# biirving/meant

Hardware: AMD Instinct MI355X
Metric: samples/sec fwd+bwd, MEANT lag=12 d=768 (higher is better)
Workload: dtype bf16; 1 GPU; full MEANT (tweet+image) fwd+CE+bwd, lag=12, d=768, 12 heads, seq=512, 224x224 p=16, E=1, vocab 64001 (BASELINE.json configs[2]/[3]); batch_per_gpu=128, global_batch=128, parallelism=dp1, micro_batches=1, train_mode_dropout=True, activation_checkpointing=False, norm_linear_fold=False, grad_allreduce=False

## Files before the change

meant_amd/csrc/qkv_fwd_by_id.hip:

```cpp
#pragma clang fp contract(off)
#include "common.h"
#include "internal.h"

#define FBYID_REQ(c, ...) MEANT_REQUIRE(c, MEANT_ERR_ARG, __VA_ARGS__)

namespace {

#include "seg_sum.h"
constexpr int PANEL = 256;

__global__ __launch_bounds__(256) void qkv_gather_kernel(const float* __restrict__ P, const int64_t* __restrict__ sorted_ids,
                                                          const int64_t* __restrict__ order, const uint8_t* __restrict__ live,
                                                          const float* __restrict__ qa, const float* __restrict__ qb,
                                                          const float* __restrict__ ka, const float* __restrict__ kb, bf16* __restrict__ qkv,
                                                          int64_t n, int N3, int D, int Dh, int R, int S, int64_t V, int cb_chunks) {
  const int lane = threadIdx.x & 63, wave = threadIdx.x >> 6;
  const int64_t s = (int64_t)blockIdx.x * 4 + wave;
  const int64_t j0 = s * SEG;
  if (j0 >= n) return;
  const int64_t j1 = j0 + SEG < n ? j0 + SEG : n;
  const int c0 = blockIdx.y * cb_chunks;
  const int left = (N3 >> 3) - c0;
  const int nch = left < cb_chunks ? left : cb_chunks;
  const bool has = lane < nch;
  const int col = (c0 + (has ? lane : 0)) * 8;
  const int sec = col / D;
  const int c = (col - sec * D) % Dh;
  const bool rot_on = qa != nullptr && sec < 2 && c < R;
  const bool kv = sec >= 1;
  const float* const tabA = (sec == 1 ? ka : qa) + (rot_on ? c : 0);
  const float* const tabB = (sec == 1 ? kb : qb) + (rot_on ? c : 0);
  long long cur = -1;
  Vec8<float> row{};

  for (int64_t jb = j0; jb < j1; jb += 64) {
    const int64_t jl = jb + lane < j1 ? jb + lane : j1 - 1;
    const long long id64 = sorted_ids[jl], ord64 = order[jl];
    const int my_id = id64 >= 0 && id64 < V ? (int)id64 : -1;
    const int my_ord = ord64 >= 0 && ord64 < n ? (int)ord64 : -1;
    const int cnt = (int)(j1 - jb < 64 ? j1 - jb : 64);
    for (int t0 = 0; t0 < cnt; t0 += 4) {
      Vec8<float> r4[4], A4[4], B4[4];
      int ord4[4];
      bool st4[4];
#pragma unroll
      for (int u = 0; u < 4; ++u) {
        const int t = t0 + u < cnt ? t0 + u : cnt - 1;
        const int id = __builtin_amdgcn_readlane(my_id, t);
        const int ord = __builtin_amdgcn_readlane(my_ord, t);
        if (id != cur) {
          cur = id;
          if (id >= 0) row = load8<float>(P + (int64_t)id * N3 + col);
        }
        r4[u] = row;
        ord4[u] = ord;
        const bool tok = t0 + u < cnt && id >= 0 && ord >= 0;
        const bool kv_ok = !live || (tok && live[ord / PANEL] != 0);
        st4[u] = tok && has && (!kv || kv_ok);
        A4[u] = Vec8<float>{};
        B4[u] = Vec8<float>{};
        if (st4[u] && rot_on) {
          const int o = (ord % S) * R;
          A4[u] = load8<float>(tabA + o);
          B4[u] = load8<float>(tabB + o);
        }
      }
#pragma unroll
      for (int u = 0; u < 4; ++u) {
        if (!st4[u]) continue;
        float v[8];
#pragma unroll
        for (int e = 0; e < 8; ++e) v[e] = r4[u].get(e);
        if (rot_on) rot_apply8(v, A4[u].lo, A4[u].hi, B4[u].lo, B4[u].hi);
        Vec8<bf16> o;
#pragma unroll
        for (int e = 0; e < 8; ++e) o.set(e, v[e]);
        store8s<bf16>(qkv + (int64_t)ord4[u] * N3 + col, o);
      }
    }
  }
}

struct FwdByIdWs { size_t ntab, rinv, p, live, total; };
FwdByIdWs fwd_byid_layout(int64_t n, int64_t d, int64_t N3, int64_t V) {
  FwdByIdWs w;
  const int64_t Vp = vpad_rows(V);
  size_t off = 0;
  const auto take = [&off](size_t bytes) { const size_t o = off; off += align256(bytes); return o; };
  w.ntab = take((size_t)Vp * d * sizeof(bf16));
  w.rinv = take((size_t)V * sizeof(float));
  w.p = take((size_t)Vp * N3 * sizeof(float));
  w.live = take((size_t)ceil_div(n, PANEL));
  w.total = off;
  return w;
}

bool fwd_byid_shape_ok(int64_t n, int64_t d, int64_t N3, int64_t V) {
  return n > 0 && d > 0 && N3 > 0 && V > 0 && n < (1ll << 31) && V < (1ll << 31) && d % 8 == 0 && N3 % 24 == 0 && N3 < (1ll << 22) && d < (1ll << 22);
}

GemmBf16Args shape_args(int64_t M, int64_t N, int64_t K) { return gemm_bf16_nt_args(nullptr, K, nullptr, nullptr, N, M, N, K); }

}

extern "C" size_t meant_qkv_embed_fwd_by_id_ws(int64_t n, int64_t d, int64_t N3, int64_t V) {
  return fwd_byid_shape_ok(n, d, N3, V) ? fwd_byid_layout(n, d, N3, V).total : 0;
}

extern "C" int meant_qkv_embed_fwd_by_id_ok(int64_t n, int64_t d, int64_t N3, int64_t V) {
  if (!fwd_byid_shape_ok(n, d, N3, V) || N3 % 3 != 0 || (N3 / 3) % 256 != 0 || n % 256 != 0) return 0;
  if (meant_num_cus() <= 0) return 0;
  const int64_t Vp = vpad_rows(V);
  return gemm_bf16_nt_streams(shape_args(n, N3, d)) && gemm_bf16_nt_streams(shape_args(Vp, N3, d)) ? 1 : 0;
}

extern "C" int meant_qkv_embed_fwd_by_id(const void* table_bf16, const float* gain, float eps, const void* w_bf16, const float* bias,
                                         const int64_t* sorted_ids, const int64_t* order, const void* kv_lists, const float* qa,
                                         const float* qb, const float* ka, const float* kb, void* qkv, int64_t n, int64_t S, int64_t d,
                                         int H, int Dh, int R, int64_t V, void* workspace, size_t workspace_bytes, void* stream) {
  FBYID_REQ(table_bf16 && gain && w_bf16 && sorted_ids && order && qkv && workspace && H > 0 && Dh > 0 && S > 0, "qkv_embed_fwd_by_id: bad argument");
  const int64_t D = (int64_t)H * Dh, N3 = 3 * D;
  MEANT_REQUIRE(fwd_byid_shape_ok(n, d, N3, V) && n % S == 0 && S < (1ll << 22) && Dh % 8 == 0, MEANT_ERR_UNSUPPORTED,
                "qkv_embed_fwd_by_id: n=%lld S=%lld d=%lld H=%d Dh=%d V=%lld: n, V < 2^31, n %% S == 0, d %% 8 == 0, Dh %% 8 == 0", (long long)n,
                (long long)S, (long long)d, H, Dh, (long long)V);
  const bool rot = qa != nullptr;
  FBYID_REQ(!rot || (qb && ka && kb && R > 0 && R % 8 == 0 && R <= Dh), "qkv_embed_fwd_by_id: bad rotary tables (rot_dim %% 8 == 0)");
  MEANT_REQUIRE(meant_qkv_embed_fwd_by_id_ok(n, d, N3, V), MEANT_ERR_UNSUPPORTED,
                "qkv_embed_fwd_by_id: the streaming NT kernel must take both the [n, H Dh] and the [V, 3 H Dh] product (n=%lld d=%lld N3=%lld V=%lld)",
                (long long)n, (long long)d, (long long)N3, (long long)V);
  const FwdByIdWs w = fwd_byid_layout(n, d, N3, V);
  MEANT_REQUIRE(workspace_bytes >= w.total, MEANT_ERR_WORKSPACE, "qkv_embed_fwd_by_id: workspace of %zu bytes needed, %zu given", w.total,
                workspace_bytes);
  FBYID_REQ(meant_aligned16(workspace) && meant_aligned16(table_bf16) && meant_aligned16(w_bf16) && meant_aligned16(qkv) &&
                (!rot || (meant_aligned16(qa) && meant_aligned16(qb) && meant_aligned16(ka) && meant_aligned16(kb))),
            "qkv_embed_fwd_by_id: 16-byte alignment");
  const bool listed = kv_lists != nullptr;
  FBYID_REQ(!listed || S % PANEL == 0, "qkv_embed_fwd_by_id: key-padding lists need S %% 256 == 0");
  hipStream_t st = (hipStream_t)stream;
  char* base = (char*)workspace;
  bf16* ntab = (bf16*)(base + w.ntab);
  float *rinv = (float*)(base + w.rinv), *P = (float*)(base + w.p);
  uint8_t* live = listed ? (uint8_t*)(base + w.live) : nullptr;
  const int64_t Vp = vpad_rows(V), nst = ceil_div(n, SEG), nblk = n / 64, npan = n / PANEL;

  const int64_t V4 = V & ~(int64_t)3;
  int rc = meant_rmsnorm_fwd(table_bf16, gain, ntab, rinv, V4, d, eps, 0.f, 0, MEANT_BF16, stream);
  if (!rc && V4 < V)
    rc = meant_rmsnorm_fwd((const bf16*)table_bf16 + (V - 4) * d, gain, ntab + (V - 4) * d, rinv + (V - 4), 4, d, eps, 0.f, 0, MEANT_BF16, stream);
  if (rc) return rc;
  hipError_t e = hipSuccess;
  if (Vp > V) e = hipMemsetAsync(ntab + V * d, 0, (size_t)(Vp - V) * d * sizeof(bf16), st);
  if (e == hipSuccess && listed) e = hipMemsetAsync(live, 0, (size_t)npan, st);
  MEANT_REQUIRE(e == hipSuccess, MEANT_ERR_LAUNCH, "qkv_embed_fwd_by_id: clearing the workspace failed: %s", hipGetErrorString(e));
  GemmBf16Args a{};
  a.A = ntab; a.lda = d; a.B = (const bf16*)w_bf16; a.ldb = d; a.C = (bf16*)P; a.ldc = N3;
  a.M = Vp; a.N = N3; a.K = d; a.bias = bias; a.epilogue = GEMM_EPI_F32_OUT;
  rc = gemm_bf16_nt_launch(a, st);
  if (rc) return rc;
  const int* const lists = (const int*)kv_lists;
  if (listed) rc = live_flags_launch(lists + MEANT_KV_LIST_HDR + nblk, lists + 1, live, npan, st);
  if (rc) return rc;
  const SegColBlocks cb = seg_col_blocks(N3, 1);
  hipLaunchKernelGGL(qkv_gather_kernel, dim3((unsigned)ceil_div(nst, 4), (unsigned)cb.ncb), dim3(256), 0, st, (const float*)P, sorted_ids, order,
                     (const uint8_t*)live, qa, qb, ka, kb, (bf16*)qkv, n, (int)N3, (int)D, Dh, rot ? R : 0, (int)S, V, cb.cb_chunks);
  MEANT_LAUNCH_CHECK("qkv_embed_fwd_by_id: gather");
  meant_route_hit(ROUTE_QKV_FWD_BY_ID);
  if (listed) return zero_panels_launch((bf16*)qkv + D, N3, 2 * D, lists + MEANT_KV_LIST_HDR + nblk + npan, lists + 2, npan, st);
  return MEANT_OK;
}
```

meant_amd/csrc/seg_sum.h:

```cpp
#pragma once

constexpr int SEG = 256;
constexpr int SEG_SHORT = 16;

struct SegAddRow {
  float* dtable; int64_t id_lo, id_hi;
  __device__ __forceinline__ bool owns(int64_t id) const { return id >= id_lo && id < id_hi; }
  __device__ __forceinline__ void put(int64_t id, int64_t ld, int64_t col, f32x4 a) const {
    f32x4* dst = reinterpret_cast<f32x4*>(dtable + id * ld + col);
    *dst = *dst + a;
  }
};
struct SegStoreHiLo {
  bf16* hi; bf16* lo;
  __device__ __forceinline__ bool owns(int64_t) const { return true; }
  __device__ __forceinline__ void put(int64_t id, int64_t ld, int64_t col, f32x4 a) const {
    bf16x4 h, l;
#pragma unroll
    for (int e = 0; e < 4; ++e) {
      h[e] = (bf16)a[e];
      l[e] = (bf16)(a[e] - (float)h[e]);
    }
    *reinterpret_cast<bf16x4*>(hi + id * ld + col) = h;
    *reinterpret_cast<bf16x4*>(lo + id * ld + col) = l;
  }
};

struct SegAllRows {
  __device__ __forceinline__ bool live(int64_t) const { return true; }
  __device__ __forceinline__ bool reads(int, bool) const { return true; }
};
template <class Store>
struct SegSlotSink {
  Store st; float* part; int64_t ld;
  __device__ __forceinline__ bool owns(int64_t id) const { return st.owns(id); }
  __device__ __forceinline__ void inside(int64_t id, int64_t col, f32x4 lo, f32x4 hi) const {
    st.put(id, ld, col, lo);
    st.put(id, ld, col + 4, hi);
  }
  __device__ __forceinline__ void cross(int64_t, int slot, int64_t col, f32x4 lo, f32x4 hi) const {
    store8<float>(part + slot * ld + col, Vec8<float>{lo, hi});
  }
};

struct SegCols { int64_t col[2]; bool has[2]; };
__device__ __forceinline__ SegCols seg_cols(int64_t width, int cb_chunks) {
  const int lane = threadIdx.x & 63;
  const int c0 = blockIdx.y * cb_chunks;
  const int left = (int)(width >> 3) - c0;
  const int nch = left < cb_chunks ? left : cb_chunks;
  return {{(int64_t)(c0 + lane) * 8, (int64_t)(c0 + lane + 64) * 8}, {lane < nch, lane + 64 < nch}};
}

template <bool COLSUM, typename T, class Rows, class Sink>
__device__ __forceinline__ void seg_walk(const T* __restrict__ src, int64_t ld, const int64_t* __restrict__ sorted_ids,
                                         const int64_t* __restrict__ order, int64_t n, int64_t V, int64_t j0, int64_t j1, const SegCols& c,
                                         const Rows& rows, const Sink& sink, float* __restrict__ csum) {
  const int lane = threadIdx.x & 63;
  float acc[2][8], cs[2][8];
#pragma unroll
  for (int e = 0; e < 8; ++e) acc[0][e] = acc[1][e] = cs[0][e] = cs[1][e] = 0.f;
  int64_t cur = sorted_ids[j0];
  bool open_left = j0 > 0 && sorted_ids[j0 - 1] == cur;

  auto flush = [&](int64_t id, int slot) {
    if (id < 0 || id >= V || !sink.owns(id)) return;
#pragma unroll
    for (int k = 0; k < 2; ++k) {
      if (!c.has[k]) continue;
      const f32x4 lo = {acc[k][0], acc[k][1], acc[k][2], acc[k][3]}, hi = {acc[k][4], acc[k][5], acc[k][6], acc[k][7]};
      if (slot < 0) sink.inside(id, c.col[k], lo, hi);
      else sink.cross(id, slot, c.col[k], lo, hi);
    }
  };

  for (int64_t jb = j0; jb < j1; jb += 64) {
    const int64_t jl = jb + lane < j1 ? jb + lane : j1 - 1;
    const long long my_id = sorted_ids[jl], my_ord = order[jl];
    const int cnt = (int)(j1 - jb < 64 ? j1 - jb : 64);
    for (int t0 = 0; t0 < cnt; t0 += 4) {
      Vec8<T> r[4][2];
      long long ids4[4];
#pragma unroll
      for (int u = 0; u < 4; ++u) {
        const int t = t0 + u < cnt ? t0 + u : cnt - 1;
        ids4[u] = __shfl(my_id, t, 64);
        const long long ord = __shfl(my_ord, t, 64);
        const bool row_ok = ord >= 0 && ord < n;
        const bool live = row_ok && rows.live(ord);
        const T* row = src + (row_ok ? ord : 0) * ld;
#pragma unroll
        for (int k = 0; k < 2; ++k) {
          r[u][k] = Vec8<T>{};
          if (c.has[k] && row_ok && rows.reads(k, live)) r[u][k] = load8s<T>(row + c.col[k]);
        }
      }
#pragma unroll
      for (int u = 0; u < 4; ++u) {
        if (t0 + u >= cnt) break;
        const int64_t id = ids4[u];
        if (id != cur) {
          flush(cur, open_left ? 0 : -1);
#pragma unroll
          for (int e = 0; e < 8; ++e) acc[0][e] = acc[1][e] = 0.f;
          cur = id;
          open_left = false;
        }
#pragma unroll
        for (int e = 0; e < 8; ++e) {
#pragma unroll
          for (int k = 0; k < 2; ++k) {
            const float a = r[u][k].get(e);
            acc[k][e] += a;
            if constexpr (COLSUM) cs[k][e] += a;
          }
        }
      }
    }
  }
  const bool open_right = j1 < n && sorted_ids[j1] == cur;
  flush(cur, open_left ? 0 : (open_right ? 1 : -1));
  if constexpr (COLSUM) {
#pragma unroll
    for (int k = 0; k < 2; ++k)
      if (c.has[k])
        store8<float>(csum + c.col[k], Vec8<float>{{cs[k][0], cs[k][1], cs[k][2], cs[k][3]}, {cs[k][4], cs[k][5], cs[k][6], cs[k][7]}});
  }
}

template <class Store>
__global__ __launch_bounds__(256) void seg_cross_kernel(const int64_t* __restrict__ sorted_ids, const float* __restrict__ part,
                                                         int* __restrict__ longk, Store st, int64_t n, int64_t d, int64_t V) {
  const int lane = threadIdx.x & 63, wave = threadIdx.x >> 6;
  const int64_t s = (int64_t)blockIdx.x * 4 + wave, j0 = s * SEG, j1 = j0 + SEG;
  if (j1 >= n) return;
  const int64_t id = sorted_ids[j1 - 1];
  const bool owner = sorted_ids[j1] == id && !(j0 > 0 && sorted_ids[j0 - 1] == id)
                     && id >= 0 && id < V && st.owns(id);
  int64_t K = 0;
  if (owner) {
    const int64_t nst = (n + SEG - 1) / SEG;
    int64_t follow = 0;
    for (int64_t t0 = s + 1;; t0 += 64) {
      const int64_t t = t0 + lane;
      const int k = __popcll(__ballot(t < nst && sorted_ids[t * SEG] == id));
      follow += k;
      if (k < 64) break;
    }
    K = follow + 1;
  }
  if (blockIdx.y == 0 && lane == 0) longk[s] = K > SEG_SHORT ? (int)K : 0;
  if (K == 0 || K > SEG_SHORT) return;
  const int64_t col = (int64_t)blockIdx.y * 256 + lane * 4;
  if (col >= d) return;
  f32x4 acc = *reinterpret_cast<const f32x4*>(part + (s * 2 + 1) * d + col);
  for (int64_t k = 1; k < K; ++k) acc += *reinterpret_cast<const f32x4*>(part + (s + k) * 2 * d + col);
  st.put(id, d, col, acc);
}

template <class Store>
__global__ __launch_bounds__(256) void seg_long_kernel(const int64_t* __restrict__ sorted_ids, const float* __restrict__ part,
                                                        const int* __restrict__ longk, Store st, int64_t d) {
  __shared__ f32x4 red[16][16];
  const int tid = threadIdx.x;
  const int64_t s = blockIdx.x;
  const int64_t K = longk[s];
  if (K == 0) return;
  const int64_t id = sorted_ids[s * SEG + SEG - 1];
  const int p = tid >> 4;
  const int64_t col = (int64_t)blockIdx.y * 64 + (tid & 15) * 4;
  const bool active = col < d;
  const int64_t piece = (K + 15) / 16, k0 = p * piece, k1 = k0 + piece < K ? k0 + piece : K;
  f32x4 acc = {0.f, 0.f, 0.f, 0.f};
  if (active) {
#pragma unroll 4
    for (int64_t k = k0; k < k1; ++k) {
      const float* row = k == 0 ? part + (s * 2 + 1) * d : part + (s + k) * 2 * d;
      acc += *reinterpret_cast<const f32x4*>(row + col);
    }
  }
  red[p][tid & 15] = acc;
  __syncthreads();
#pragma unroll
  for (int h = 8; h > 0; h >>= 1) {
    if (p < h) red[p][tid & 15] += red[p + h][tid & 15];
    __syncthreads();
  }
  if (p == 0 && active) st.put(id, d, col, red[0][tid & 15]);
}

struct SegColBlocks { int ncb, cb_chunks; };
inline SegColBlocks seg_col_blocks(int64_t width, int per_lane) {
  const int64_t chunks = width >> 3, ncb = ceil_div(chunks, 64 * per_lane);
  return {(int)ncb, (int)ceil_div(chunks, ncb)};
}

template <class Store>
void seg_cross_launch(const Store& store, const int64_t* sorted_ids, const float* part, int* longk, int64_t n, int64_t d, int64_t V,
                      hipStream_t st) {
  const int64_t nst = ceil_div(n, SEG);
  if (nst <= 1) return;
  hipLaunchKernelGGL(seg_cross_kernel<Store>, dim3((unsigned)ceil_div(nst - 1, 4), (unsigned)ceil_div(d, 256)), dim3(256), 0, st, sorted_ids,
                     part, longk, store, n, d, V);
  hipLaunchKernelGGL(seg_long_kernel<Store>, dim3((unsigned)(nst - 1), (unsigned)ceil_div(d, 64)), dim3(256), 0, st, sorted_ids, part,
                     (const int*)longk, store, d);
}
```

Baseline: 3812 samples/s.

## Software-pipeline gather and segment-sum walks with double-buffered loads

Restructures the QKV gather kernel and the shared seg_walk helper into a software pipeline. The next group of row loads, and the index block after that, are requested before the current group is stored or accumulated, with liveness flags precomputed per lane. The gather gains a specialised no-rotary path with unconditional row loads, uses segment indices made wave-uniform, and rounds column blocks to multiples of 8. The intent is to hide global-load latency in these memory-bound gather and reduce passes, at the cost of more registers and branchless dummy loads.

```diff
diff --git a/meant_amd/csrc/qkv_fwd_by_id.hip b/meant_amd/csrc/qkv_fwd_by_id.hip
--- a/meant_amd/csrc/qkv_fwd_by_id.hip
+++ b/meant_amd/csrc/qkv_fwd_by_id.hip
@@ -8,6 +8,101 @@
 
 #include "seg_sum.h"
 constexpr int PANEL = 256;
+
+constexpr int GATHER_G = 2;
+struct GatherBlock { int id, ord, off, kv_ok; };
+template <bool ROT>
+struct GatherSet;
+template <>
+struct GatherSet<true> { Vec8<float> r[GATHER_G], A[GATHER_G], B[GATHER_G]; int ord[GATHER_G]; bool st[GATHER_G]; };
+template <>
+struct GatherSet<false> { Vec8<float> r[GATHER_G]; int ord[GATHER_G]; bool st[GATHER_G]; };
+inline SegColBlocks gather_col_blocks(int64_t width) {
+  const SegColBlocks cb = seg_col_blocks(width, 1);
+  const int cut = (cb.cb_chunks + 7) & ~7;
+  return {(int)ceil_div(width >> 3, cut), cut};
+}
+
+template <bool ROT>
+__device__ __forceinline__ void gather_walk(const float* __restrict__ P, const int64_t* __restrict__ sorted_ids, const int64_t* __restrict__ order,
+                                            const uint8_t* __restrict__ live, const float* __restrict__ tabA, const float* __restrict__ tabB,
+                                            bf16* __restrict__ qkv, int64_t n, int N3, int R, int S, int64_t V, int64_t j0, int64_t j1, int col,
+                                            bool has, bool kv, bool rot_on) {
+  const int lane = threadIdx.x & 63;
+  int cur = -1;
+  Vec8<float> row{};
+
+  auto entries = [&](int64_t jb) {
+    const int64_t jl = jb + lane < j1 ? jb + lane : j1 - 1;
+    const long long id64 = sorted_ids[jl], ord64 = order[jl];
+    GatherBlock b;
+    b.id = id64 >= 0 && id64 < V ? (int)id64 : -1;
+    b.ord = ord64 >= 0 && ord64 < n ? (int)ord64 : -1;
+    b.off = b.ord >= 0 ? (b.ord % S) * R : 0;
+    b.kv_ok = 1;
+    return b;
+  };
+  auto flags = [&](const GatherBlock& b) { return !live || (b.ord >= 0 && live[b.ord / PANEL] != 0) ? 1 : 0; };
+  auto request = [&](const GatherBlock& b, int t0, int cnt, GatherSet<ROT>& g) {
+#pragma unroll
+    for (int u = 0; u < GATHER_G; ++u) {
+      const int t = t0 + u < cnt ? t0 + u : (cnt ? cnt - 1 : 0);
+      const int id = __builtin_amdgcn_readlane(b.id, t);
+      const int ord = __builtin_amdgcn_readlane(b.ord, t);
+      g.ord[u] = ord;
+      g.st[u] = t0 + u < cnt && id >= 0 && ord >= 0 && has && (!kv || __builtin_amdgcn_readlane(b.kv_ok, t) != 0);
+      if constexpr (ROT) {
+        if (id != cur) {
+          cur = id;
+          if (id >= 0) row = load8<float>(P + (int64_t)id * N3 + col);
+        }
+        g.r[u] = row;
+        const int o = __builtin_amdgcn_readlane(b.off, t);
+        g.A[u] = load8<float>(tabA + o);
+        g.B[u] = load8<float>(tabB + o);
+      } else {
+        g.r[u] = load8<float>(P + (int64_t)(id >= 0 ? id : 0) * N3 + col);
+      }
+    }
+  };
+  auto store = [&](const GatherSet<ROT>& g) {
+#pragma unroll
+    for (int u = 0; u < GATHER_G; ++u) {
+      if (!g.st[u]) continue;
+      float v[8];
+#pragma unroll
+      for (int e = 0; e < 8; ++e) v[e] = g.r[u].get(e);
+      if constexpr (ROT) {
+        if (rot_on) rot_apply8(v, g.A[u].lo, g.A[u].hi, g.B[u].lo, g.B[u].hi);
+      }
+      Vec8<bf16> o;
+#pragma unroll
+      for (int e = 0; e < 8; ++e) o.set(e, v[e]);
+      store8s<bf16>(qkv + (int64_t)g.ord[u] * N3 + col, o);
+    }
+  };
+
+  GatherSet<ROT> ga, gb;
+  GatherBlock blk = entries(j0), nxt = entries(j0 + 64);
+  blk.kv_ok = flags(blk);
+  request(blk, 0, (int)(j1 - j0 < 64 ? j1 - j0 : 64), ga);
+  for (int64_t jb = j0; jb < j1; jb += 64) {
+    const int cnt = (int)(j1 - jb < 64 ? j1 - jb : 64);
+    const int ncnt = jb + 64 < j1 ? (int)(j1 - jb - 64 < 64 ? j1 - jb - 64 : 64) : 0;
+    const GatherBlock after = entries(jb + 128);
+    nxt.kv_ok = flags(nxt);
+    for (int t0 = 0; t0 < cnt; t0 += 2 * GATHER_G) {
+      request(blk, t0 + GATHER_G, cnt, gb);
+      store(ga);
+      const bool last = t0 + 2 * GATHER_G >= cnt;
+      const GatherBlock from{last ? nxt.id : blk.id, last ? nxt.ord : blk.ord, last ? nxt.off : blk.off, last ? nxt.kv_ok : blk.kv_ok};
+      request(from, last ? 0 : t0 + 2 * GATHER_G, last ? ncnt : cnt, ga);
+      store(gb);
+    }
+    blk = nxt;
+    nxt = after;
+  }
+}
 
 __global__ __launch_bounds__(256) void qkv_gather_kernel(const float* __restrict__ P, const int64_t* __restrict__ sorted_ids,
                                                           const int64_t* __restrict__ order, const uint8_t* __restrict__ live,
@@ -15,7 +110,7 @@
                                                           const float* __restrict__ ka, const float* __restrict__ kb, bf16* __restrict__ qkv,
                                                           int64_t n, int N3, int D, int Dh, int R, int S, int64_t V, int cb_chunks) {
   const int lane = threadIdx.x & 63, wave = threadIdx.x >> 6;
-  const int64_t s = (int64_t)blockIdx.x * 4 + wave;
+  const int64_t s = seg_uniform64((int64_t)blockIdx.x * 4 + wave);
   const int64_t j0 = s * SEG;
   if (j0 >= n) return;
   const int64_t j1 = j0 + SEG < n ? j0 + SEG : n;
@@ -28,57 +123,16 @@
   const int c = (col - sec * D) % Dh;
   const bool rot_on = qa != nullptr && sec < 2 && c < R;
   const bool kv = sec >= 1;
-  const float* const tabA = (sec == 1 ? ka : qa) + (rot_on ? c : 0);
-  const float* const tabB = (sec == 1 ? kb : qb) + (rot_on ? c : 0);
-  long long cur = -1;
-  Vec8<float> row{};
-
-  for (int64_t jb = j0; jb < j1; jb += 64) {
-    const int64_t jl = jb + lane < j1 ? jb + lane : j1 - 1;
-    const long long id64 = sorted_ids[jl], ord64 = order[jl];
-    const int my_id = id64 >= 0 && id64 < V ? (int)id64 : -1;
-    const int my_ord = ord64 >= 0 && ord64 < n ? (int)ord64 : -1;
-    const int cnt = (int)(j1 - jb < 64 ? j1 - jb : 64);
-    for (int t0 = 0; t0 < cnt; t0 += 4) {
-      Vec8<float> r4[4], A4[4], B4[4];
-      int ord4[4];
-      bool st4[4];
-#pragma unroll
-      for (int u = 0; u < 4; ++u) {
-        const int t = t0 + u < cnt ? t0 + u : cnt - 1;
-        const int id = __builtin_amdgcn_readlane(my_id, t);
-        const int ord = __builtin_amdgcn_readlane(my_ord, t);
-        if (id != cur) {
-          cur = id;
-          if (id >= 0) row = load8<float>(P + (int64_t)id * N3 + col);
-        }
-        r4[u] = row;
-        ord4[u] = ord;
-        const bool tok = t0 + u < cnt && id >= 0 && ord >= 0;
-        const bool kv_ok = !live || (tok && live[ord / PANEL] != 0);
-        st4[u] = tok && has && (!kv || kv_ok);
-        A4[u] = Vec8<float>{};
-        B4[u] = Vec8<float>{};
-        if (st4[u] && rot_on) {
-          const int o = (ord % S) * R;
-          A4[u] = load8<float>(tabA + o);
-          B4[u] = load8<float>(tabB + o);
-        }
-      }
-#pragma unroll
-      for (int u = 0; u < 4; ++u) {
-        if (!st4[u]) continue;
-        float v[8];
-#pragma unroll
-        for (int e = 0; e < 8; ++e) v[e] = r4[u].get(e);
-        if (rot_on) rot_apply8(v, A4[u].lo, A4[u].hi, B4[u].lo, B4[u].hi);
-        Vec8<bf16> o;
-#pragma unroll
-        for (int e = 0; e < 8; ++e) o.set(e, v[e]);
-        store8s<bf16>(qkv + (int64_t)ord4[u] * N3 + col, o);
-      }
-    }
+  const unsigned long long rot_lanes = __ballot(rot_on);
+  if (rot_lanes == 0) {
+    gather_walk<false>(P, sorted_ids, order, live, nullptr, nullptr, qkv, n, N3, R, S, V, j0, j1, col, has, kv, false);
+    return;
   }
+  const int first = __builtin_ctzll(rot_lanes);
+  const int rsec = __builtin_amdgcn_readlane(sec, first), rc = __builtin_amdgcn_readlane(c, first);
+  const float* const tabA = (rot_on ? (sec == 1 ? ka : qa) + c : (rsec == 1 ? ka : qa) + rc);
+  const float* const tabB = (rot_on ? (sec == 1 ? kb : qb) + c : (rsec == 1 ? kb : qb) + rc);
+  gather_walk<true>(P, sorted_ids, order, live, tabA, tabB, qkv, n, N3, R, S, V, j0, j1, col, has, kv, rot_on);
 }
 
 struct FwdByIdWs { size_t ntab, rinv, p, live, total; };
@@ -160,7 +214,7 @@
   const int* const lists = (const int*)kv_lists;
   if (listed) rc = live_flags_launch(lists + MEANT_KV_LIST_HDR + nblk, lists + 1, live, npan, st);
   if (rc) return rc;
-  const SegColBlocks cb = seg_col_blocks(N3, 1);
+  const SegColBlocks cb = gather_col_blocks(N3);
   hipLaunchKernelGGL(qkv_gather_kernel, dim3((unsigned)ceil_div(nst, 4), (unsigned)cb.ncb), dim3(256), 0, st, (const float*)P, sorted_ids, order,
                      (const uint8_t*)live, qa, qb, ka, kb, (bf16*)qkv, n, (int)N3, (int)D, Dh, rot ? R : 0, (int)S, V, cb.cb_chunks);
   MEANT_LAUNCH_CHECK("qkv_embed_fwd_by_id: gather");
diff --git a/meant_amd/csrc/seg_sum.h b/meant_amd/csrc/seg_sum.h
--- a/meant_amd/csrc/seg_sum.h
+++ b/meant_amd/csrc/seg_sum.h
@@ -43,20 +43,35 @@
   }
 };
 
-struct SegCols { int64_t col[2]; bool has[2]; };
+struct SegCols { int64_t col[2]; bool has[2]; int64_t first; };
 __device__ __forceinline__ SegCols seg_cols(int64_t width, int cb_chunks) {
   const int lane = threadIdx.x & 63;
   const int c0 = blockIdx.y * cb_chunks;
   const int left = (int)(width >> 3) - c0;
   const int nch = left < cb_chunks ? left : cb_chunks;
-  return {{(int64_t)(c0 + lane) * 8, (int64_t)(c0 + lane + 64) * 8}, {lane < nch, lane + 64 < nch}};
-}
+  return {{(int64_t)(c0 + lane) * 8, (int64_t)(c0 + lane + 64) * 8}, {lane < nch, lane + 64 < nch}, (int64_t)c0 * 8};
+}
+
+__device__ __forceinline__ long long seg_uniform64(long long v) {
+  const unsigned lo = __builtin_amdgcn_readfirstlane((int)(unsigned)v), hi = __builtin_amdgcn_readfirstlane((int)(v >> 32));
+  return (long long)(((unsigned long long)hi << 32) | lo);
+}
+__device__ __forceinline__ long long seg_lane64(long long v, int t) {
+  const unsigned lo = __builtin_amdgcn_readlane((int)(unsigned)v, t), hi = __builtin_amdgcn_readlane((int)(v >> 32), t);
+  return (long long)(((unsigned long long)hi << 32) | lo);
+}
+
+struct SegBlock { long long id, ord; int flags; };
+constexpr int SEG_ROW_OK = 1, SEG_ROW_LIVE = 2;
+template <typename T>
+struct SegSet { Vec8<T> r[4][2]; bool on[4][2]; long long id[4]; };
 
 template <bool COLSUM, typename T, class Rows, class Sink>
 __device__ __forceinline__ void seg_walk(const T* __restrict__ src, int64_t ld, const int64_t* __restrict__ sorted_ids,
-                                         const int64_t* __restrict__ order, int64_t n, int64_t V, int64_t j0, int64_t j1, const SegCols& c,
+                                         const int64_t* __restrict__ order, int64_t n, int64_t V, int64_t j0_, int64_t j1_, const SegCols& c,
                                          const Rows& rows, const Sink& sink, float* __restrict__ csum) {
   const int lane = threadIdx.x & 63;
+  const int64_t j0 = seg_uniform64(j0_), j1 = seg_uniform64(j1_);
   float acc[2][8], cs[2][8];
 #pragma unroll
   for (int e = 0; e < 8; ++e) acc[0][e] = acc[1][e] = cs[0][e] = cs[1][e] = 0.f;
@@ -74,49 +89,74 @@
     }
   };
 
-  for (int64_t jb = j0; jb < j1; jb += 64) {
+  auto entries = [&](int64_t jb) {
     const int64_t jl = jb + lane < j1 ? jb + lane : j1 - 1;
-    const long long my_id = sorted_ids[jl], my_ord = order[jl];
-    const int cnt = (int)(j1 - jb < 64 ? j1 - jb : 64);
-    for (int t0 = 0; t0 < cnt; t0 += 4) {
-      Vec8<T> r[4][2];
-      long long ids4[4];
-#pragma unroll
-      for (int u = 0; u < 4; ++u) {
-        const int t = t0 + u < cnt ? t0 + u : cnt - 1;
-        ids4[u] = __shfl(my_id, t, 64);
-        const long long ord = __shfl(my_ord, t, 64);
-        const bool row_ok = ord >= 0 && ord < n;
-        const bool live = row_ok && rows.live(ord);
-        const T* row = src + (row_ok ? ord : 0) * ld;
-#pragma unroll
-        for (int k = 0; k < 2; ++k) {
-          r[u][k] = Vec8<T>{};
-          if (c.has[k] && row_ok && rows.reads(k, live)) r[u][k] = load8s<T>(row + c.col[k]);
+    return SegBlock{sorted_ids[jl], order[jl], 0};
+  };
+  auto flags = [&](const SegBlock& b) {
+    const bool row_ok = b.ord >= 0 && b.ord < n;
+    return !row_ok ? 0 : (rows.live(b.ord) ? SEG_ROW_OK | SEG_ROW_LIVE : SEG_ROW_OK);
+  };
+  auto request = [&](const SegBlock& b, int t0, int cnt, SegSet<T>& g) {
+#pragma unroll
+    for (int u = 0; u < 4; ++u) {
+      const int t = t0 + u < cnt ? t0 + u : cnt - 1;
+      g.id[u] = seg_lane64(b.id, t);
+      const long long ord = seg_lane64(b.ord, t);
+      const int fl = __builtin_amdgcn_readlane(b.flags, t);
+      const bool row_ok = (fl & SEG_ROW_OK) != 0, live = (fl & SEG_ROW_LIVE) != 0;
+      const T* row = src + (row_ok ? ord : 0) * ld;
+#pragma unroll
+      for (int k = 0; k < 2; ++k) {
+        g.on[u][k] = row_ok && rows.reads(k, live);
+        g.r[u][k] = load8s<T>(c.has[k] && g.on[u][k] ? row + c.col[k] : src + c.first);
+      }
+    }
+  };
+  auto add = [&](int t0, int cnt, const SegSet<T>& g) {
+#pragma unroll
+    for (int u = 0; u < 4; ++u) {
+      if (t0 + u >= cnt) break;
+      const int64_t id = g.id[u];
+      if (id != cur) {
+        flush(cur, open_left ? 0 : -1);
+#pragma unroll
+        for (int e = 0; e < 8; ++e) acc[0][e] = acc[1][e] = 0.f;
+        cur = id;
+        open_left = false;
+      }
+#pragma unroll
+      for (int k = 0; k < 2; ++k) {
+        const Vec8<T> v = g.on[u][k] ? g.r[u][k] : Vec8<T>{};
+#pragma unroll
+        for (int e = 0; e < 8; ++e) {
+          const float a = v.get(e);
+          acc[k][e] += a;
+          if constexpr (COLSUM) cs[k][e] += a;
         }
       }
-#pragma unroll
-      for (int u = 0; u < 4; ++u) {
-        if (t0 + u >= cnt) break;
-        const int64_t id = ids4[u];
-        if (id != cur) {
-          flush(cur, open_left ? 0 : -1);
-#pragma unroll
-          for (int e = 0; e < 8; ++e) acc[0][e] = acc[1][e] = 0.f;
-          cur = id;
-          open_left = false;
-        }
-#pragma unroll
-        for (int e = 0; e < 8; ++e) {
-#pragma unroll
-          for (int k = 0; k < 2; ++k) {
-            const float a = r[u][k].get(e);
-            acc[k][e] += a;
-            if constexpr (COLSUM) cs[k][e] += a;
-          }
-        }
-      }
-    }
+    }
+  };
+
+  SegSet<T> ga, gb;
+  SegBlock blk = entries(j0), nxt = entries(j0 + 64);
+  blk.flags = flags(blk);
+  request(blk, 0, (int)(j1 - j0 < 64 ? j1 - j0 : 64), ga);
+  for (int64_t jb = j0; jb < j1; jb += 64) {
+    const int cnt = (int)(j1 - jb < 64 ? j1 - jb : 64);
+    const int ncnt = jb + 64 < j1 ? (int)(j1 - jb - 64 < 64 ? j1 - jb - 64 : 64) : 1;
+    const SegBlock after = entries(jb + 128);
+    nxt.flags = flags(nxt);
+    for (int t0 = 0; t0 < cnt; t0 += 8) {
+      request(blk, t0 + 4, cnt, gb);
+      add(t0, cnt, ga);
+      const bool last = t0 + 8 >= cnt;
+      const SegBlock from{last ? nxt.id : blk.id, last ? nxt.ord : blk.ord, last ? nxt.flags : blk.flags};
+      request(from, last ? 0 : t0 + 8, last ? ncnt : cnt, ga);
+      add(t0 + 4, cnt, gb);
+    }
+    blk = nxt;
+    nxt = after;
   }
   const bool open_right = j1 < n && sorted_ids[j1] == cur;
   flush(cur, open_left ? 0 : (open_right ? 1 : -1));
```

Measured after the change: 3852 samples/s (median of 6 runs). +1.1%, better.
